# fraunhoferhhi/gaussian_gan_decoder

Measured on AMD Instinct MI355X. Metric: forward raster frames/s, 1M Gaussians @ 1024x1024, higher is better.
Workload: dtype f32; 1 GPU; 1000000 synthetic Gaussians ('cube' scene, seed 0, SH degree 0), 1024x1024, forward raster fp32, inputs resident in HBM; num_rendered=4152095, tiles=4096, parallelism=scene-parallel x1 (no collective)

## Files before the change

gaussian_gan_decoder_amd/csrc/ggd_lookback.inc:

```
constexpr uint32_t STATUS_PUB = 1u << 30, STATUS_COUNT_MASK = STATUS_PUB - 1u;
constexpr int LOOKBACK_BATCH = 16;

__device__ __forceinline__ uint32_t status_load(uint32_t* p) {
  return __hip_atomic_load(p, __ATOMIC_RELAXED, __HIP_MEMORY_SCOPE_AGENT);
}
__device__ __forceinline__ void status_store(uint32_t* p, uint32_t v) {
  __hip_atomic_store(p, v, __ATOMIC_RELAXED, __HIP_MEMORY_SCOPE_AGENT);
}

template <int STRIDE>
__device__ __forceinline__ uint32_t lookback_sum(uint32_t* p, int cnt) {
  uint32_t acc = 0;
  for (int b0 = 0; b0 < cnt; b0 += LOOKBACK_BATCH) {
    uint32_t v[LOOKBACK_BATCH];
#pragma unroll
    for (int i = 0; i < LOOKBACK_BATCH; ++i) v[i] = (b0 + i < cnt) ? status_load(p + (size_t)(b0 + i) * STRIDE) : STATUS_PUB;
#pragma unroll
    for (int i = 0; i < LOOKBACK_BATCH; ++i) {
      uint32_t x = v[i];
      if ((x >> 30) == 0u) {
        uint32_t* q = p + (size_t)(b0 + i) * STRIDE;
        do { __builtin_amdgcn_s_sleep(1); x = status_load(q); } while ((x >> 30) == 0u);
      }
      acc += x & STATUS_COUNT_MASK;
    }
  }
  return acc;
}

template <int STRIDE, typename TileT>
__device__ __forceinline__ uint32_t lookback_two_level(uint32_t* status, int col, int rows, TileT tile, int gshift, uint32_t local,
                                                       uint32_t start) {
  const int grp = (int)(tile >> gshift), mem = (int)(tile & (((TileT)1 << gshift) - (TileT)1));
  uint32_t* tile_words = status + col;
  uint32_t* group_words = status + (size_t)rows * STRIDE + col;
  status_store(tile_words + (size_t)tile * STRIDE, STATUS_PUB | local);
  const uint32_t in_group = lookback_sum<STRIDE>(tile_words + ((size_t)grp << gshift) * STRIDE, mem);
  if (mem == (1 << gshift) - 1) {
    const uint32_t aggregate = STATUS_PUB | (in_group + local);
    status_store(group_words + (size_t)grp * STRIDE, aggregate);
  }
  return start + in_group + lookback_sum<STRIDE>(group_words, grp);
}
```

gaussian_gan_decoder_amd/csrc/ggd_rowbin.hip:

```cpp
#include "ggd_common.h"

namespace {

#include "ggd_scan.inc"
#include "ggd_lookback.inc"

constexpr int RB_WAVES = RB_THREADS / 64;
constexpr int RB_STAGE = 4096;
constexpr int RB_STAGE1 = 4096;
constexpr int RB_WCHUNK = 64 * RB_IPL;

__device__ __forceinline__ void rb_write_row_tables(uint32_t* tab, int lane, uint32_t tot, uint32_t inc, uint32_t ent_cap) {
  const uint32_t rs = inc - tot;
  tab[RB_TAB_ROWSTART + lane] = rs;
  if (lane == 63) tab[RB_TAB_ROWSTART + 64] = inc;
  const uint32_t have = rs < ent_cap ? min(tot, ent_cap - rs) : 0u;
  const uint32_t nblk = (have + RB_CHUNK - 1) / RB_CHUNK;
  const uint32_t binc = wave_inclusive_scan(nblk);
  tab[RB_TAB_ROWBLK + lane] = binc - nblk;
  if (lane == 63) tab[RB_TAB_ROWBLK + 64] = binc;
  tab[RB_TAB_FLAG + lane] = 0u;
}

__global__ __launch_bounds__(RB_THREADS) void rb_count1_kernel(int W, int H, const uint2* __restrict__ rect,
                                                               const uint32_t* __restrict__ order,
                                                               const uint32_t* __restrict__ n_vis_ptr, int P,
                                                               uint2* __restrict__ packed, uint32_t* __restrict__ counts1,
                                                               const uint32_t* __restrict__ order_alt,
                                                               const uint32_t* __restrict__ use_alt) {
  __shared__ int diff[65];
  if (use_alt && *use_alt != 0u) order = order_alt;
  const uint32_t n_vis = min((uint32_t)P, *n_vis_ptr);
  const uint32_t base = (uint32_t)blockIdx.x * RB_CHUNK;
  if (base >= n_vis) return;
  const int tid = threadIdx.x;
  if (tid < 65) diff[tid] = 0;
  __syncthreads();
#pragma unroll
  for (int q = 0; q < RB_IPL; ++q) {
    const uint32_t rnk = base + (uint32_t)q * RB_THREADS + tid;
    if (rnk < n_vis) {
      const uint32_t id = order[rnk];
      const uint2 rc = rect[id];
      int x0 = (int)(rc.x & 0xffffu), x1 = (int)(rc.x >> 16), y0 = (int)(rc.y & 0xffffu), y1 = (int)(rc.y >> 16);
      const int n = (x1 - x0) * (y1 - y0);
      if (n <= 0) { x0 = x1 = y0 = y1 = 0; }
      packed[rnk] = make_uint2(id, (uint32_t)x0 | ((uint32_t)x1 << 8) | ((uint32_t)y0 << 16) | ((uint32_t)y1 << 24));
      if (n > 0) { atomicAdd(&diff[y0], 1); atomicAdd(&diff[y1], -1); }
    }
  }
  __syncthreads();
  if (tid < 64) counts1[(size_t)blockIdx.x * 64 + tid] = (uint32_t)wave_inclusive_scan(diff[tid]);
}

__global__ __launch_bounds__(1024) void rb_scan1_kernel(uint32_t* __restrict__ counts1,
                                                        const uint32_t* __restrict__ n_vis_ptr, int P,
                                                        uint32_t* __restrict__ tab, uint32_t ent_cap) {
  __shared__ uint32_t part[16][64];
  const int lane = threadIdx.x & 63, wv = threadIdx.x >> 6;
  const uint32_t n_vis = min((uint32_t)P, *n_vis_ptr);
  const int nb = (int)((n_vis + RB_CHUNK - 1) / RB_CHUNK);
  const int per = (nb + 15) / 16;
  const int r0 = min(nb, wv * per), r1 = min(nb, r0 + per);
  uint32_t s = 0;
#pragma unroll 8
  for (int r = r0; r < r1; ++r) s += counts1[(size_t)r * 64 + lane];
  part[wv][lane] = s;
  __syncthreads();
  uint32_t run = 0, tot = 0;
#pragma unroll
  for (int w = 0; w < 16; ++w) { const uint32_t p = part[w][lane]; if (w < wv) run += p; tot += p; }
#pragma unroll 8
  for (int r = r0; r < r1; ++r) {
    const size_t idx = (size_t)r * 64 + lane;
    const uint32_t c = counts1[idx];
    counts1[idx] = run;
    run += c;
  }
  if (wv == 0) rb_write_row_tables(tab, lane, tot, wave_inclusive_scan(tot), ent_cap);
}

template <int D, uint32_t M>
__device__ __forceinline__ void tr_stage(uint32_t& lo, uint32_t& hi, uint32_t lane) {
  const bool up = (lane & (uint32_t)D) != 0;
  const uint32_t keep = up ? ~M : M;
  const uint32_t slo = up ? ((lo & M) << D) : ((lo & ~M) >> D);
  const uint32_t shi = up ? ((hi & M) << D) : ((hi & ~M) >> D);
  lo = (lo & keep) | (uint32_t)__shfl_xor((int)slo, D, 64);
  hi = (hi & keep) | (uint32_t)__shfl_xor((int)shi, D, 64);
}

__device__ __forceinline__ uint64_t wave_transpose64(uint64_t row) {
  const uint32_t lane = threadIdx.x & 63;
  uint32_t lo = (uint32_t)row, hi = (uint32_t)(row >> 32);
  {
    const bool up = (lane & 32u) != 0;
    const uint32_t recv = (uint32_t)__shfl_xor((int)(up ? lo : hi), 32, 64);
    if (up) lo = recv; else hi = recv;
  }
  tr_stage<16, 0x0000FFFFu>(lo, hi, lane);
  tr_stage<8, 0x00FF00FFu>(lo, hi, lane);
  tr_stage<4, 0x0F0F0F0Fu>(lo, hi, lane);
  tr_stage<2, 0x33333333u>(lo, hi, lane);
  tr_stage<1, 0x55555555u>(lo, hi, lane);
  return (uint64_t)lo | ((uint64_t)hi << 32);
}

__device__ __forceinline__ uint32_t wave_cols(const uint32_t (&iv)[RB_IPL], int n_items, uint64_t (&cols)[RB_IPL]) {
  uint32_t cnt = 0;
#pragma unroll
  for (int q = 0; q < RB_IPL; ++q) {
    cols[q] = 0ull;
    if (q * 64 >= n_items) continue;
    const uint32_t l = iv[q] & 0xffu, h = iv[q] >> 8;
    const uint64_t below_h = h >= 64u ? ~0ull : ((1ull << h) - 1ull);
    const uint64_t row = h > l ? (below_h & ~((1ull << l) - 1ull)) : 0ull;
    cols[q] = wave_transpose64(row);
    cnt += (uint32_t)__popcll(cols[q]);
  }
  return cnt;
}

__device__ __forceinline__ bool rb_walk_items(uint32_t width, uint32_t fill) {
  const int wi = __ballot(width > 16u) ? 3 : (__ballot(width > 8u) ? 2 : (__ballot(width > 4u) ? 1 : 0));
  const int wf = __ballot(fill > 16u) ? 3 : (__ballot(fill > 8u) ? 2 : (__ballot(fill > 4u) ? 1 : 0));
  return wi <= wf + 1;
}

template <bool TWO, typename Emit>
__device__ __forceinline__ void wave_emit(const uint32_t (&iv)[RB_IPL], const uint32_t (&pa)[RB_IPL],
                                          const uint32_t (&pb)[RB_IPL], const uint64_t (&cols)[RB_IPL], int n_items,
                                          uint32_t& dst, uint4* slab , Emit&& emit) {
  const int lane = threadIdx.x & 63;
  const uint64_t lt_mask = (1ull << lane) - 1ull;
#pragma unroll
  for (int q = 0; q < RB_IPL; ++q) {
    if (q * 64 >= n_items) continue;
    __builtin_amdgcn_wave_barrier();
    slab[lane] = make_uint4((uint32_t)cols[q], (uint32_t)(cols[q] >> 32), dst, 0u);
    __builtin_amdgcn_wave_barrier();
    const uint32_t l = iv[q] & 0xffu, h = iv[q] >> 8;
    if (rb_walk_items(h > l ? h - l : 0u, (uint32_t)__popcll(cols[q]))) {
      for (uint32_t b = l; __ballot(b < h) != 0ull; ++b) {
        const bool act = b < h;
        const uint4 e = slab[act ? b : 0u];
        const uint64_t m = (uint64_t)e.x | ((uint64_t)e.y << 32);
        if (act) emit(e.z + (uint32_t)__popcll(m & lt_mask), pa[q], TWO ? pb[q] : 0u);
      }
      dst += (uint32_t)__popcll(cols[q]);
    } else {
      uint64_t col = cols[q];
      while (__ballot(col != 0ull) != 0ull) {
        const bool act = col != 0ull;
        const int k = act ? (__ffsll((unsigned long long)col) - 1) : 0;
        col &= col - 1ull;
        const uint32_t a = (uint32_t)__shfl((int)pa[q], k, 64);
        const uint32_t bb = TWO ? (uint32_t)__shfl((int)pb[q], k, 64) : 0u;
        if (act) { emit(dst, a, bb); dst += 1; }
      }
    }
  }
}

__global__ __launch_bounds__(RB_THREADS) void rb_scatter1_kernel(const uint2* __restrict__ packed,
                                                                 const uint32_t* __restrict__ n_vis_ptr, int P,
                                                                 const uint32_t* __restrict__ prefix1,
                                                                 const uint32_t* __restrict__ tab,
                                                                 uint2* __restrict__ ent, uint32_t ent_cap) {
  __shared__ uint4 slab[RB_WAVES][64];
  __shared__ uint32_t wcnt[RB_WAVES][64];
  const uint32_t n_vis = min((uint32_t)P, *n_vis_ptr);
  const uint32_t base = (uint32_t)blockIdx.x * RB_CHUNK;
  if (base >= n_vis) return;
  const int tid = threadIdx.x, lane = tid & 63, wv = tid >> 6;
  const uint32_t wbeg = base + (uint32_t)wv * RB_WCHUNK;
  const int n_items = (int)min((uint32_t)RB_WCHUNK, n_vis > wbeg ? n_vis - wbeg : 0u);
  uint32_t iv[RB_IPL], pa[RB_IPL], pb[RB_IPL];
#pragma unroll
  for (int q = 0; q < RB_IPL; ++q) {
    const int i = q * 64 + lane;
    uint2 it = make_uint2(0, 0);
    if (i < n_items) it = packed[wbeg + i];
    pa[q] = it.x; pb[q] = it.y & 0xffffu;
    iv[q] = it.y >> 16;
  }
  uint64_t cols[RB_IPL];
  const uint32_t mine = wave_cols(iv, n_items, cols);
  wcnt[wv][lane] = mine;
  __syncthreads();
  uint32_t dst = tab[RB_TAB_ROWSTART + lane] + prefix1[(size_t)blockIdx.x * 64 + lane];
#pragma unroll
  for (int w = 0; w < RB_WAVES; ++w) if (w < wv) dst += wcnt[w][lane];
  wave_emit<true>(iv, pa, pb, cols, n_items, dst, slab[wv], [&](uint32_t d, uint32_t id, uint32_t xx) {
    if (d < ent_cap) ent[d] = make_uint2(id, xx);
  });
}

__global__ __launch_bounds__(RB_THREADS) void rb_level1_kernel(const uint2* __restrict__ rect, const uint32_t* __restrict__ order,
                                                               const uint32_t* __restrict__ n_vis_ptr, int P,
                                                               const uint32_t* __restrict__ rowtot, uint32_t* status,
                                                               int chunks_max, int gshift_max, uint32_t* __restrict__ tab,
                                                               uint2* __restrict__ ent, uint32_t ent_cap,
                                                               const uint32_t* __restrict__ order_alt,
                                                               const uint32_t* __restrict__ use_alt,
                                                               const uint32_t* __restrict__ rowinst) {
  __shared__ uint4 slab[RB_WAVES][64];
  __shared__ uint32_t wcnt[RB_WAVES][64];
  __shared__ uint32_t s_base[64];
  __shared__ uint2 stage[RB_STAGE1];
  if (use_alt && *use_alt != 0u) order = order_alt;
  const uint32_t n_vis = min((uint32_t)P, *n_vis_ptr);
  const int tid = threadIdx.x, lane = tid & 63, wv = tid >> 6;
  uint32_t rowstart = 0;
  if (wv == 0) {
    uint32_t tot = 0;
#pragma unroll
    for (int r = 0; r < GGD_FOLD_REPS; ++r) tot += rowtot[r * 64 + lane];
    const uint32_t inc = wave_inclusive_scan(tot);
    rowstart = inc - tot;
    if (blockIdx.x == 0) {
      rb_write_row_tables(tab, lane, tot, inc, ent_cap);
      if (rowinst) {
        uint32_t inst = 0;
#pragma unroll
        for (int r = 0; r < GGD_FOLD_REPS; ++r) inst += rowinst[r * 64 + lane];
        tab[RB_TAB_ROWINST + lane] = inst;
      }
    }
  }
  const uint32_t base = (uint32_t)blockIdx.x * RB_CHUNK;
  if (base >= n_vis) return;
  const uint32_t wbeg = base + (uint32_t)wv * RB_WCHUNK;
  const int n_items = (int)min((uint32_t)RB_WCHUNK, n_vis > wbeg ? n_vis - wbeg : 0u);
  uint32_t iv[RB_IPL], pa[RB_IPL], pb[RB_IPL];
#pragma unroll
  for (int q = 0; q < RB_IPL; ++q) {
    const int i = q * 64 + lane;
    pa[q] = 0; pb[q] = 0; iv[q] = 0;
    if (i < n_items) {
      const uint32_t id = order[wbeg + i];
      const uint2 rc = rect[id];
      const uint32_t x0 = rc.x & 0xffffu, x1 = rc.x >> 16, y0 = rc.y & 0xffffu, y1 = rc.y >> 16;
      pa[q] = id;
      if ((int)(x1 - x0) * (int)(y1 - y0) > 0) { pb[q] = x0 | (x1 << 8); iv[q] = y0 | (y1 << 8); }
    }
  }
  uint64_t cols[RB_IPL];
  const uint32_t mine = wave_cols(iv, n_items, cols);
  wcnt[wv][lane] = mine;
  __syncthreads();
  if (wv == 0) {
    const uint32_t local = wcnt[0][lane] + wcnt[1][lane] + wcnt[2][lane] + wcnt[3][lane];
    const int chunk = (int)blockIdx.x;
    const int live = (int)((n_vis + RB_CHUNK - 1) / RB_CHUNK);
    const int gs = min(ggd_group_shift(live), gshift_max);
    s_base[lane] = lookback_two_level<64>(status, lane, chunks_max, chunk, gs, local, rowstart);
  }
  __syncthreads();
  uint32_t before = 0, rowtot_c = 0;
#pragma unroll
  for (int w = 0; w < RB_WAVES; ++w) { const uint32_t c = wcnt[w][lane]; if (w < wv) before += c; rowtot_c += c; }
  const uint32_t rowend = wave_inclusive_scan(rowtot_c);
  const uint32_t total = (uint32_t)__shfl((int)rowend, 63, 64);
  const uint32_t rowbeg = rowend - rowtot_c;
  const uint32_t gbase = s_base[lane];
  if (total <= (uint32_t)RB_STAGE1) {
    uint32_t ldst = rowbeg + before;
    wave_emit<true>(iv, pa, pb, cols, n_items, ldst, slab[wv], [&](uint32_t d, uint32_t id, uint32_t xx) { stage[d] = make_uint2(id, xx); });
    __syncthreads();
#pragma unroll 4
    for (int c = wv; c < 64; c += RB_WAVES) {
      const uint32_t n = (uint32_t)__shfl((int)rowtot_c, c, 64);
      if (n == 0) continue;
      const uint32_t b0 = (uint32_t)__shfl((int)rowbeg, c, 64), g = (uint32_t)__shfl((int)gbase, c, 64);
      for (uint32_t k = lane; k < n; k += 64) {
        const uint32_t d = g + k;
        if (d < ent_cap) ent[d] = stage[b0 + k];
      }
    }
    return;
  }
  uint32_t dst = gbase + before;
  wave_emit<true>(iv, pa, pb, cols, n_items, dst, slab[wv], [&](uint32_t d, uint32_t id, uint32_t xx) {
    if (d < ent_cap) ent[d] = make_uint2(id, xx);
  });
}

__device__ __forceinline__ bool rb_block_row_range(const uint32_t* __restrict__ tab, uint32_t blk, uint32_t ent_cap, int& row,
                                                   uint32_t& chunk, uint32_t& rbeg, uint32_t& rend) {
  const int lane = threadIdx.x & 63;
  const uint32_t first = tab[RB_TAB_ROWBLK + lane];
  const uint32_t total = tab[RB_TAB_ROWBLK + 64];
  const uint32_t start = tab[RB_TAB_ROWSTART + lane];
  const uint32_t all = tab[RB_TAB_ROWSTART + 64];
  if (blk >= total) return false;
  const int r = __popcll(__ballot(first <= blk)) - 1;
  row = r; chunk = blk - (uint32_t)__shfl((int)first, r, 64);
  rbeg = (uint32_t)__shfl((int)start, r, 64);
  rend = min(r == 63 ? all : (uint32_t)__shfl((int)start, (r + 1) & 63, 64), ent_cap);
  return true;
}

__global__ __launch_bounds__(RB_THREADS) void rb_count2_kernel(const uint2* __restrict__ ent, uint32_t ent_cap,
                                                               const uint32_t* __restrict__ tab,
                                                               uint32_t* __restrict__ counts2) {
  __shared__ int diff[65];
  int row; uint32_t chunk, rbeg, rend;
  if (!rb_block_row_range(tab, blockIdx.x, ent_cap, row, chunk, rbeg, rend)) return;
  const int tid = threadIdx.x;
  const uint32_t base = rbeg + chunk * RB_CHUNK;
  uint32_t xs[RB_IPL];
#pragma unroll
  for (int q = 0; q < RB_IPL; ++q) {
    const uint32_t i = base + (uint32_t)q * RB_THREADS + tid;
    xs[q] = i < rend ? ent[i].y : 0u;
  }
  if (tid < 65) diff[tid] = 0;
  __syncthreads();
#pragma unroll
  for (int q = 0; q < RB_IPL; ++q) {
    const uint32_t x0 = xs[q] & 0xffu, x1 = (xs[q] >> 8) & 0xffu;
    if (x1 > x0) { atomicAdd(&diff[x0], 1); atomicAdd(&diff[x1], -1); }
  }
  __syncthreads();
  if (tid < 64) counts2[(size_t)blockIdx.x * 64 + tid] = (uint32_t)wave_inclusive_scan(diff[tid]);
}

__global__ __launch_bounds__(1024) void rb_scan2_kernel(uint32_t* __restrict__ counts2, uint32_t* tab, int gx, int gy,
                                                        uint32_t* __restrict__ ranges) {
  __shared__ uint32_t part[16][64];
  const int lane = threadIdx.x & 63, wv = threadIdx.x >> 6;
  const int r = blockIdx.x;
  const uint32_t b0 = tab[RB_TAB_ROWBLK + r], b1 = tab[RB_TAB_ROWBLK + r + 1];
  const uint32_t nb = b1 - b0, per = (nb + 15u) / 16u;
  const uint32_t c0 = b0 + min(nb, (uint32_t)wv * per), c1 = min(b1, c0 + per);
  uint32_t s = 0;
#pragma unroll 4
  for (uint32_t b = c0; b < c1; ++b) s += counts2[(size_t)b * 64 + lane];
  part[wv][lane] = s;
  __syncthreads();
  uint32_t run = 0, tot = 0;
#pragma unroll
  for (int w = 0; w < 16; ++w) { const uint32_t p = part[w][lane]; if (w < wv) run += p; tot += p; }
#pragma unroll 4
  for (uint32_t b = c0; b < c1; ++b) {
    const size_t idx = (size_t)b * 64 + lane;
    const uint32_t c = counts2[idx];
    counts2[idx] = run;
    run += c;
  }
  if (wv == 0) {
    const uint32_t inc = wave_inclusive_scan(tot);
    if (lane == 63) {
      tab[RB_TAB_ROWINST + r] = inc;
      __builtin_amdgcn_fence(__ATOMIC_RELEASE, "agent");
      __hip_atomic_store(&tab[RB_TAB_FLAG + r], 1u, __ATOMIC_RELAXED, __HIP_MEMORY_SCOPE_AGENT);
    }
    uint32_t below = 0;
    if (lane < r) {
      while (__hip_atomic_load(&tab[RB_TAB_FLAG + lane], __ATOMIC_RELAXED, __HIP_MEMORY_SCOPE_AGENT) == 0u) {}
    }
    __builtin_amdgcn_fence(__ATOMIC_ACQUIRE, "agent");
    if (lane < r) below = __hip_atomic_load(&tab[RB_TAB_ROWINST + lane], __ATOMIC_RELAXED, __HIP_MEMORY_SCOPE_AGENT);
    const uint32_t binc = wave_inclusive_scan(below);
    const uint32_t rowbase = (uint32_t)__builtin_amdgcn_readlane((int)binc, 63);
    if (lane < gx) {
      const uint32_t start = rowbase + inc - tot;
      tab[RB_TAB_TILESTART + r * 64 + lane] = start;
      const int t = r * gx + lane;
      ranges[2 * t] = tot ? start : 0u;
      ranges[2 * t + 1] = tot ? start + tot : 0u;
    }
  }
}

template <bool SCAN>
__global__ __launch_bounds__(RB_THREADS) void rb_scatter2_kernel(const uint2* __restrict__ ent, uint32_t ent_cap,
                                                                 const uint32_t* __restrict__ tab,
                                                                 const uint32_t* __restrict__ prefix2,
                                                                 uint32_t* __restrict__ list, uint32_t capacity,
                                                                 uint32_t main_blocks, ggd_scan_piggy pg, int gx, int gy,
                                                                 uint32_t* __restrict__ ranges) {
  __shared__ uint4 slab[RB_WAVES][64];
  __shared__ uint32_t wcnt[RB_WAVES][64];
  __shared__ __attribute__((aligned(16))) uint32_t wsum[SCAN ? 2 * RB_WAVES : 1][64];
  __shared__ uint32_t stage[RB_STAGE];
  if (blockIdx.x >= main_blocks) {
    scan_apply_block(pg.in, pg.out, pg.n, pg.block_sums, (int)(blockIdx.x - main_blocks), stage, pg.sum_stride);
    return;
  }
  const int tid = threadIdx.x, lane = tid & 63, wv = tid >> 6;
  uint32_t rowinst = 0, rowblks = 0;
  if constexpr (SCAN) {
    rowinst = tab[RB_TAB_ROWINST + lane];
    rowblks = tab[RB_TAB_ROWBLK + lane + 1] - tab[RB_TAB_ROWBLK + lane];
    if ((int)blockIdx.x < gy && wv == 0) {
      const uint32_t nb_z = (uint32_t)__shfl((int)rowblks, (int)blockIdx.x, 64);
      if (nb_z == 0u && lane < gx) {
        const int t = (int)blockIdx.x * gx + lane;
        ranges[2 * t] = 0u;
        ranges[2 * t + 1] = 0u;
      }
    }
  }
  int row; uint32_t chunk, rbeg, rend;
  if (!rb_block_row_range(tab, blockIdx.x, ent_cap, row, chunk, rbeg, rend)) return;
  const uint32_t wbeg = rbeg + chunk * RB_CHUNK + (uint32_t)wv * RB_WCHUNK;
  const int n_items = (int)min((uint32_t)RB_WCHUNK, rend > wbeg ? rend - wbeg : 0u);
  uint32_t iv[RB_IPL], pa[RB_IPL], pb[RB_IPL];
  const uint32_t blkbeg = rbeg + chunk * RB_CHUNK;
  uint2 raw[RB_IPL];
#pragma unroll
  for (int q = 0; q < RB_IPL; ++q) {
    const int i = q * 64 + lane;
    raw[q] = ent[i < n_items ? wbeg + (uint32_t)i : blkbeg];
  }
  uint32_t gbase = 0;
  if constexpr (SCAN) {
    const uint32_t blk0 = blockIdx.x - chunk;
    const uint32_t nblk_row = (uint32_t)__shfl((int)rowblks, row, 64);
    constexpr int BATCH = 8;
    const uint32_t sub = (uint32_t)lane >> 4, c4 = ((uint32_t)lane & 15u) * 4u;
    uint4 bef4 = make_uint4(0, 0, 0, 0), tot4 = make_uint4(0, 0, 0, 0);
    for (uint32_t k0 = (uint32_t)wv * 4u; k0 < nblk_row; k0 += 4u * RB_WAVES * BATCH) {
      uint4 v[BATCH];
#pragma unroll
      for (int j = 0; j < BATCH; ++j) {
        const uint32_t k = k0 + sub + (uint32_t)(4 * RB_WAVES * j);
        v[j] = make_uint4(0, 0, 0, 0);
        if (k < nblk_row) v[j] = *reinterpret_cast<const uint4*>(prefix2 + (size_t)(blk0 + k) * 64 + c4);
      }
#pragma unroll
      for (int j = 0; j < BATCH; ++j) {
        const uint32_t k = k0 + sub + (uint32_t)(4 * RB_WAVES * j);
        tot4.x += v[j].x; tot4.y += v[j].y; tot4.z += v[j].z; tot4.w += v[j].w;
        const uint32_t m = k < chunk ? 0xffffffffu : 0u;
        bef4.x += v[j].x & m; bef4.y += v[j].y & m; bef4.z += v[j].z & m; bef4.w += v[j].w & m;
      }
    }
#pragma unroll
    for (int d = 16; d <= 32; d <<= 1) {
      tot4.x += (uint32_t)__shfl_xor((int)tot4.x, d, 64); tot4.y += (uint32_t)__shfl_xor((int)tot4.y, d, 64);
      tot4.z += (uint32_t)__shfl_xor((int)tot4.z, d, 64); tot4.w += (uint32_t)__shfl_xor((int)tot4.w, d, 64);
      bef4.x += (uint32_t)__shfl_xor((int)bef4.x, d, 64); bef4.y += (uint32_t)__shfl_xor((int)bef4.y, d, 64);
      bef4.z += (uint32_t)__shfl_xor((int)bef4.z, d, 64); bef4.w += (uint32_t)__shfl_xor((int)bef4.w, d, 64);
    }
    if (lane < 16) {
      *reinterpret_cast<uint4*>(&wsum[wv][c4]) = bef4;
      *reinterpret_cast<uint4*>(&wsum[RB_WAVES + wv][c4]) = tot4;
    }
  } else {
    gbase = tab[RB_TAB_TILESTART + row * 64 + lane] + prefix2[(size_t)blockIdx.x * 64 + lane];
  }
#pragma unroll
  for (int q = 0; q < RB_IPL; ++q) {
    const bool have = q * 64 + lane < n_items;
    pa[q] = have ? raw[q].x : 0u; pb[q] = 0;
    iv[q] = have ? raw[q].y & 0xffffu : 0u;
  }
  uint64_t cols[RB_IPL];
  const uint32_t mine = wave_cols(iv, n_items, cols);
  wcnt[wv][lane] = mine;
  __syncthreads();
  if constexpr (SCAN) {
    uint32_t bef = 0, tot = 0;
#pragma unroll
    for (int w = 0; w < RB_WAVES; ++w) { bef += wsum[w][lane]; tot += wsum[RB_WAVES + w][lane]; }
    const uint32_t rinc = wave_inclusive_scan(rowinst);
    const uint32_t rowbase = (uint32_t)__shfl((int)(rinc - rowinst), row, 64);
    const uint32_t start = rowbase + wave_inclusive_scan(tot) - tot;
    gbase = start + bef;
    if (chunk == 0u && wv == 0 && lane < gx) {
      const int t = row * gx + lane;
      ranges[2 * t] = tot ? start : 0u;
      ranges[2 * t + 1] = tot ? start + tot : 0u;
    }
  }
  uint32_t before = 0, coltot = 0;
#pragma unroll
  for (int w = 0; w < RB_WAVES; ++w) { const uint32_t c = wcnt[w][lane]; if (w < wv) before += c; coltot += c; }
  const uint32_t colend = wave_inclusive_scan(coltot);
  const uint32_t total = (uint32_t)__shfl((int)colend, 63, 64);
  const uint32_t colbeg = colend - coltot;
  if (total <= (uint32_t)RB_STAGE) {
    uint32_t ldst = colbeg + before;
    wave_emit<false>(iv, pa, pb, cols, n_items, ldst, slab[wv], [&](uint32_t d, uint32_t id, uint32_t) { stage[d] = id; });
    __syncthreads();
#pragma unroll 4
    for (int c = wv; c < 64; c += RB_WAVES) {
      const uint32_t n = (uint32_t)__shfl((int)coltot, c, 64);
      if (n == 0) continue;
      const uint32_t b0 = (uint32_t)__shfl((int)colbeg, c, 64), g = (uint32_t)__shfl((int)gbase, c, 64);
      for (uint32_t k = lane; k < n; k += 64) {
        const uint32_t d = g + k;
        if (d < capacity) list[d] = stage[b0 + k];
      }
    }
    return;
  }
  uint32_t dst = gbase + before;
  wave_emit<false>(iv, pa, pb, cols, n_items, dst, slab[wv], [&](uint32_t d, uint32_t id, uint32_t) {
    if (d < capacity) list[d] = id;
  });
}

#include "ggd_rowbin_wide.inc"

}

bool ggd_rowbin_supported(int W, int H) { return W > 0 && H > 0 && (W + 15) / 16 <= 255 && (H + 15) / 16 <= 255; }

int ggd_launch_rowbin(ggd_ctx* ctx, hipStream_t s, const ggd_params& prm, const uint2* rect, const uint32_t* order,
                      const uint32_t* n_vis_ptr, uint32_t* list, uint32_t* ranges, uint32_t capacity, void* tmp,
                      size_t tmp_bytes, const uint32_t* order_alt, const uint32_t* use_alt, const ggd_scan_piggy* apply,
                      const uint32_t* fold_rowtot, uint32_t* fold_status1, const uint32_t* fold_rowinst, bool* scan_in_scatter) {
  if (scan_in_scatter) *scan_in_scatter = false;
  if (!ggd_rowbin_supported(prm.width, prm.height)) return ggd_fail(ctx, GGD_E_INVALID, "tile grid too large for row binning");
  const ggd_rowbin_tmp lay = ggd_rowbin_layout(prm.P, capacity, prm.width, prm.height);
  if (tmp_bytes < lay.total) return ggd_fail(ctx, GGD_E_INVALID, "rowbin tmp too small");
  const int gx = (prm.width + 15) / 16, gy = (prm.height + 15) / 16;
  const bool wide = rb_is_wide(prm.width, prm.height);
  char* p = static_cast<char*>(tmp);
  uint2* packed = reinterpret_cast<uint2*>(p + lay.packed);
  uint32_t* counts1 = reinterpret_cast<uint32_t*>(p + lay.counts1);
  uint32_t* tab = reinterpret_cast<uint32_t*>(p + lay.tab);
  uint2* ent = reinterpret_cast<uint2*>(p + lay.ent);
  uint32_t* counts2 = reinterpret_cast<uint32_t*>(p + lay.counts2);
  const int nb1 = rb_blocks1(prm.P);
  const uint32_t nb2 = rb_blocks2(capacity, wide);
  const uint32_t nb_apply = apply ? (uint32_t)apply->nb : 0u;
  const ggd_scan_piggy pg = apply ? *apply : ggd_scan_piggy{};
  static_assert(RB_THREADS == SCAN_THREADS, "the appended scan workgroups share the launch's block size");
  if (wide) {
    const int ngy = (gy + 63) / 64, ngx = (gx + 63) / 64, nby = 64 * ngy, nbx = 64 * ngx;
    hipLaunchKernelGGL(rbw_count1_kernel, dim3(nb1), dim3(RB_THREADS), 0, s, rect, order, n_vis_ptr, prm.P, nby, packed,
                       counts1, order_alt, use_alt);
    hipLaunchKernelGGL(rbw_scan1_kernel, dim3(1), dim3(1024), 0, s, counts1, n_vis_ptr, prm.P, ngy, tab, capacity);
    hipLaunchKernelGGL(rbw_scatter1_kernel, dim3(nb1), dim3(RB_THREADS), 0, s, packed, n_vis_ptr, prm.P, ngy, counts1, tab,
                       ent, capacity);
    hipLaunchKernelGGL(rbw_count2_kernel, dim3(nb2), dim3(RB_THREADS), 0, s, ent, capacity, tab, nbx, counts2);
    hipLaunchKernelGGL(rbw_scan2_kernel, dim3(gy), dim3(1024), 0, s, counts2, tab, gx, gy, ngx, ranges);
    hipLaunchKernelGGL(rbw_scatter2_kernel, dim3(nb2 + nb_apply), dim3(RB_THREADS), 0, s, ent, capacity, tab, ngx, counts2, list,
                       capacity, nb2, pg);
    GGD_HIP(hipGetLastError());
    return GGD_OK;
  }
  const bool fused2 = fold_rowtot && fold_status1 && fold_rowinst && nb2 <= RB_SCAN_IN_SCATTER_MAX_BLOCKS;
  if (fold_rowtot && fold_status1) {
    hipLaunchKernelGGL(rb_level1_kernel, dim3(nb1), dim3(RB_THREADS), 0, s, rect, order, n_vis_ptr, prm.P, fold_rowtot,
                       fold_status1, nb1, ggd_group_shift(nb1), tab, ent, capacity, order_alt, use_alt,
                       fused2 ? fold_rowinst : nullptr);
  } else {
    hipLaunchKernelGGL(rb_count1_kernel, dim3(nb1), dim3(RB_THREADS), 0, s, prm.width, prm.height, rect, order,
                       n_vis_ptr, prm.P, packed, counts1, order_alt, use_alt);
    hipLaunchKernelGGL(rb_scan1_kernel, dim3(1), dim3(1024), 0, s, counts1, n_vis_ptr, prm.P, tab, capacity);
    hipLaunchKernelGGL(rb_scatter1_kernel, dim3(nb1), dim3(RB_THREADS), 0, s, packed, n_vis_ptr, prm.P, counts1, tab,
                       ent, capacity);
  }
  hipLaunchKernelGGL(rb_count2_kernel, dim3(nb2), dim3(RB_THREADS), 0, s, ent, capacity, tab, counts2);
  if (fused2) {
    hipLaunchKernelGGL(rb_scatter2_kernel<true>, dim3(nb2 + nb_apply), dim3(RB_THREADS), 0, s, ent, capacity, tab, counts2, list,
                       capacity, nb2, pg, gx, gy, ranges);
    if (scan_in_scatter) *scan_in_scatter = true;
  } else {
    hipLaunchKernelGGL(rb_scan2_kernel, dim3(gy), dim3(1024), 0, s, counts2, tab, gx, gy, ranges);
    hipLaunchKernelGGL(rb_scatter2_kernel<false>, dim3(nb2 + nb_apply), dim3(RB_THREADS), 0, s, ent, capacity, tab, counts2, list,
                       capacity, nb2, pg, gx, gy, ranges);
  }
  GGD_HIP(hipGetLastError());
  return GGD_OK;
}
```

Measured before the change: 5122 frames/s.

## Overlap decoupled lookback with staging emit in rowbin level-1 kernel

Splits the two-level lookback so each block publishes its own group prefix early, issues the loads for earlier group aggregates, and only settles them after emitting entries into shared staging. This hides the lookback latency behind the emit work. The change also hoists the order/rect loads ahead of the row-table scan, moves the early-exit path to the top, and batches the staging-to-global copy loop four rows at a time using readlane. Risks: more register pressure from the held aggregate batch and the prefetched rects, and a subtle ordering dependency on publishing before waiting.

```diff
diff --git a/gaussian_gan_decoder_amd/csrc/ggd_lookback.inc b/gaussian_gan_decoder_amd/csrc/ggd_lookback.inc
--- a/gaussian_gan_decoder_amd/csrc/ggd_lookback.inc
+++ b/gaussian_gan_decoder_amd/csrc/ggd_lookback.inc
@@ -9,28 +9,48 @@
 }
 
 template <int STRIDE>
+__device__ __forceinline__ void lookback_request(uint32_t* p, int cnt, int b0, uint32_t (&v)[LOOKBACK_BATCH]) {
+#pragma unroll
+  for (int i = 0; i < LOOKBACK_BATCH; ++i) v[i] = (b0 + i < cnt) ? status_load(p + (size_t)(b0 + i) * STRIDE) : STATUS_PUB;
+}
+template <int STRIDE>
+__device__ __forceinline__ uint32_t lookback_settle(uint32_t* p, int b0, const uint32_t (&v)[LOOKBACK_BATCH]) {
+  uint32_t acc = 0;
+#pragma unroll
+  for (int i = 0; i < LOOKBACK_BATCH; ++i) {
+    uint32_t x = v[i];
+    if ((x >> 30) == 0u) {
+      uint32_t* q = p + (size_t)(b0 + i) * STRIDE;
+      do { __builtin_amdgcn_s_sleep(1); x = status_load(q); } while ((x >> 30) == 0u);
+    }
+    acc += x & STATUS_COUNT_MASK;
+  }
+  return acc;
+}
+template <int STRIDE>
 __device__ __forceinline__ uint32_t lookback_sum(uint32_t* p, int cnt) {
   uint32_t acc = 0;
   for (int b0 = 0; b0 < cnt; b0 += LOOKBACK_BATCH) {
     uint32_t v[LOOKBACK_BATCH];
-#pragma unroll
-    for (int i = 0; i < LOOKBACK_BATCH; ++i) v[i] = (b0 + i < cnt) ? status_load(p + (size_t)(b0 + i) * STRIDE) : STATUS_PUB;
-#pragma unroll
-    for (int i = 0; i < LOOKBACK_BATCH; ++i) {
-      uint32_t x = v[i];
-      if ((x >> 30) == 0u) {
-        uint32_t* q = p + (size_t)(b0 + i) * STRIDE;
-        do { __builtin_amdgcn_s_sleep(1); x = status_load(q); } while ((x >> 30) == 0u);
-      }
-      acc += x & STATUS_COUNT_MASK;
-    }
+    lookback_request<STRIDE>(p, cnt, b0, v);
+    acc += lookback_settle<STRIDE>(p, b0, v);
   }
+  return acc;
+}
+template <int STRIDE>
+__device__ __forceinline__ uint32_t lookback_sum_finish(uint32_t* p, int cnt, uint32_t (&v)[LOOKBACK_BATCH]) {
+  uint32_t acc = 0;
+  int b0 = 0;
+  do {
+    if (b0 != 0) lookback_request<STRIDE>(p, cnt, b0, v);
+    acc += lookback_settle<STRIDE>(p, b0, v);
+    b0 += LOOKBACK_BATCH;
+  } while (b0 < cnt);
   return acc;
 }
 
 template <int STRIDE, typename TileT>
-__device__ __forceinline__ uint32_t lookback_two_level(uint32_t* status, int col, int rows, TileT tile, int gshift, uint32_t local,
-                                                       uint32_t start) {
+__device__ __forceinline__ uint32_t lookback_own_group(uint32_t* status, int col, int rows, TileT tile, int gshift, uint32_t local) {
   const int grp = (int)(tile >> gshift), mem = (int)(tile & (((TileT)1 << gshift) - (TileT)1));
   uint32_t* tile_words = status + col;
   uint32_t* group_words = status + (size_t)rows * STRIDE + col;
@@ -40,5 +60,25 @@
     const uint32_t aggregate = STATUS_PUB | (in_group + local);
     status_store(group_words + (size_t)grp * STRIDE, aggregate);
   }
-  return start + in_group + lookback_sum<STRIDE>(group_words, grp);
+  return in_group;
 }
+template <int STRIDE, typename TileT>
+__device__ __forceinline__ void lookback_groups_request(uint32_t* status, int col, int rows, TileT tile, int gshift,
+                                                        uint32_t (&v)[LOOKBACK_BATCH]) {
+  lookback_request<STRIDE>(status + (size_t)rows * STRIDE + col, (int)(tile >> gshift), 0, v);
+}
+template <int STRIDE, typename TileT>
+__device__ __forceinline__ uint32_t lookback_groups_finish(uint32_t* status, int col, int rows, TileT tile, int gshift,
+                                                           uint32_t (&v)[LOOKBACK_BATCH]) {
+  return lookback_sum_finish<STRIDE>(status + (size_t)rows * STRIDE + col, (int)(tile >> gshift), v);
+}
+template <int STRIDE, typename TileT>
+__device__ __forceinline__ uint32_t lookback_earlier_groups(uint32_t* status, int col, int rows, TileT tile, int gshift) {
+  return lookback_sum<STRIDE>(status + (size_t)rows * STRIDE + col, (int)(tile >> gshift));
+}
+template <int STRIDE, typename TileT>
+__device__ __forceinline__ uint32_t lookback_two_level(uint32_t* status, int col, int rows, TileT tile, int gshift, uint32_t local,
+                                                       uint32_t start) {
+  const uint32_t in_group = lookback_own_group<STRIDE>(status, col, rows, tile, gshift, local);
+  return start + in_group + lookback_earlier_groups<STRIDE>(status, col, rows, tile, gshift);
+}
diff --git a/gaussian_gan_decoder_amd/csrc/ggd_rowbin.hip b/gaussian_gan_decoder_amd/csrc/ggd_rowbin.hip
--- a/gaussian_gan_decoder_amd/csrc/ggd_rowbin.hip
+++ b/gaussian_gan_decoder_amd/csrc/ggd_rowbin.hip
@@ -208,79 +208,126 @@
   __shared__ uint32_t wcnt[RB_WAVES][64];
   __shared__ uint32_t s_base[64];
   __shared__ uint2 stage[RB_STAGE1];
-  if (use_alt && *use_alt != 0u) order = order_alt;
-  const uint32_t n_vis = min((uint32_t)P, *n_vis_ptr);
-  const int tid = threadIdx.x, lane = tid & 63, wv = tid >> 6;
+  const uint32_t nv_word = *n_vis_ptr;
+  const uint32_t alt_word = *(use_alt ? use_alt : n_vis_ptr);
+  asm volatile("" : : "s"(nv_word), "s"(alt_word));
+  if (use_alt && alt_word != 0u) order = order_alt;
+  const uint32_t n_vis = min((uint32_t)P, nv_word);
+  const int tid = threadIdx.x, lane = tid & 63, wv = __builtin_amdgcn_readfirstlane(tid >> 6);
+  const uint32_t base = (uint32_t)blockIdx.x * RB_CHUNK;
+  if (base >= n_vis) {
+    if (blockIdx.x == 0 && wv == 0) {
+      uint32_t tot = 0, inst = 0;
+#pragma unroll
+      for (int r = 0; r < GGD_FOLD_REPS; ++r) tot += rowtot[r * 64 + lane];
+      rb_write_row_tables(tab, lane, tot, wave_inclusive_scan(tot), ent_cap);
+      if (rowinst) {
+#pragma unroll
+        for (int r = 0; r < GGD_FOLD_REPS; ++r) inst += rowinst[r * 64 + lane];
+        tab[RB_TAB_ROWINST + lane] = inst;
+      }
+    }
+    return;
+  }
+  const uint32_t wbeg = base + (uint32_t)wv * RB_WCHUNK;
+  const int n_items = (int)min((uint32_t)RB_WCHUNK, n_vis > wbeg ? n_vis - wbeg : 0u);
+  const bool tables = blockIdx.x == 0;
+  uint32_t rt[GGD_FOLD_REPS], ri[GGD_FOLD_REPS];
+  if (wv == 0) {
+#pragma unroll
+    for (int r = 0; r < GGD_FOLD_REPS; ++r) rt[r] = rowtot[r * 64 + lane];
+    if (tables && rowinst) {
+#pragma unroll
+      for (int r = 0; r < GGD_FOLD_REPS; ++r) ri[r] = rowinst[r * 64 + lane];
+    }
+  }
+  uint32_t ids[RB_IPL];
+  uint2 rcs[RB_IPL];
+#pragma unroll
+  for (int q = 0; q < RB_IPL; ++q) ids[q] = order[min(wbeg + (uint32_t)(q * 64 + lane), n_vis - 1u)];
+#pragma unroll
+  for (int q = 0; q < RB_IPL; ++q) rcs[q] = rect[ids[q]];
   uint32_t rowstart = 0;
   if (wv == 0) {
     uint32_t tot = 0;
 #pragma unroll
-    for (int r = 0; r < GGD_FOLD_REPS; ++r) tot += rowtot[r * 64 + lane];
+    for (int r = 0; r < GGD_FOLD_REPS; ++r) tot += rt[r];
     const uint32_t inc = wave_inclusive_scan(tot);
     rowstart = inc - tot;
-    if (blockIdx.x == 0) {
+    if (tables) {
       rb_write_row_tables(tab, lane, tot, inc, ent_cap);
       if (rowinst) {
         uint32_t inst = 0;
 #pragma unroll
-        for (int r = 0; r < GGD_FOLD_REPS; ++r) inst += rowinst[r * 64 + lane];
+        for (int r = 0; r < GGD_FOLD_REPS; ++r) inst += ri[r];
         tab[RB_TAB_ROWINST + lane] = inst;
       }
     }
   }
-  const uint32_t base = (uint32_t)blockIdx.x * RB_CHUNK;
-  if (base >= n_vis) return;
-  const uint32_t wbeg = base + (uint32_t)wv * RB_WCHUNK;
-  const int n_items = (int)min((uint32_t)RB_WCHUNK, n_vis > wbeg ? n_vis - wbeg : 0u);
   uint32_t iv[RB_IPL], pa[RB_IPL], pb[RB_IPL];
 #pragma unroll
   for (int q = 0; q < RB_IPL; ++q) {
-    const int i = q * 64 + lane;
-    pa[q] = 0; pb[q] = 0; iv[q] = 0;
-    if (i < n_items) {
-      const uint32_t id = order[wbeg + i];
-      const uint2 rc = rect[id];
-      const uint32_t x0 = rc.x & 0xffffu, x1 = rc.x >> 16, y0 = rc.y & 0xffffu, y1 = rc.y >> 16;
-      pa[q] = id;
-      if ((int)(x1 - x0) * (int)(y1 - y0) > 0) { pb[q] = x0 | (x1 << 8); iv[q] = y0 | (y1 << 8); }
-    }
+    const bool have = q * 64 + lane < n_items;
+    const uint32_t x0 = rcs[q].x & 0xffffu, x1 = rcs[q].x >> 16, y0 = rcs[q].y & 0xffffu, y1 = rcs[q].y >> 16;
+    const bool area = have && (int)(x1 - x0) * (int)(y1 - y0) > 0;
+    pa[q] = have ? ids[q] : 0u;
+    pb[q] = area ? x0 | (x1 << 8) : 0u;
+    iv[q] = area ? y0 | (y1 << 8) : 0u;
   }
   uint64_t cols[RB_IPL];
   const uint32_t mine = wave_cols(iv, n_items, cols);
   wcnt[wv][lane] = mine;
   __syncthreads();
-  if (wv == 0) {
-    const uint32_t local = wcnt[0][lane] + wcnt[1][lane] + wcnt[2][lane] + wcnt[3][lane];
-    const int chunk = (int)blockIdx.x;
-    const int live = (int)((n_vis + RB_CHUNK - 1) / RB_CHUNK);
-    const int gs = min(ggd_group_shift(live), gshift_max);
-    s_base[lane] = lookback_two_level<64>(status, lane, chunks_max, chunk, gs, local, rowstart);
-  }
-  __syncthreads();
   uint32_t before = 0, rowtot_c = 0;
 #pragma unroll
   for (int w = 0; w < RB_WAVES; ++w) { const uint32_t c = wcnt[w][lane]; if (w < wv) before += c; rowtot_c += c; }
+  const int chunk = (int)blockIdx.x;
+  const int live = (int)((n_vis + RB_CHUNK - 1) / RB_CHUNK);
+  const int gs = min(ggd_group_shift(live), gshift_max);
+  uint32_t in_group = 0;
+  if (wv == 0) in_group = lookback_own_group<64>(status, lane, chunks_max, chunk, gs, rowtot_c);
   const uint32_t rowend = wave_inclusive_scan(rowtot_c);
   const uint32_t total = (uint32_t)__shfl((int)rowend, 63, 64);
   const uint32_t rowbeg = rowend - rowtot_c;
-  const uint32_t gbase = s_base[lane];
   if (total <= (uint32_t)RB_STAGE1) {
+    uint32_t agg[LOOKBACK_BATCH];
+    if (wv == 0) lookback_groups_request<64>(status, lane, chunks_max, chunk, gs, agg);
     uint32_t ldst = rowbeg + before;
     wave_emit<true>(iv, pa, pb, cols, n_items, ldst, slab[wv], [&](uint32_t d, uint32_t id, uint32_t xx) { stage[d] = make_uint2(id, xx); });
+    if (wv == 0) s_base[lane] = rowstart + in_group + lookback_groups_finish<64>(status, lane, chunks_max, chunk, gs, agg);
     __syncthreads();
-#pragma unroll 4
-    for (int c = wv; c < 64; c += RB_WAVES) {
-      const uint32_t n = (uint32_t)__shfl((int)rowtot_c, c, 64);
-      if (n == 0) continue;
-      const uint32_t b0 = (uint32_t)__shfl((int)rowbeg, c, 64), g = (uint32_t)__shfl((int)gbase, c, 64);
-      for (uint32_t k = lane; k < n; k += 64) {
-        const uint32_t d = g + k;
-        if (d < ent_cap) ent[d] = stage[b0 + k];
+    const uint32_t gbase = s_base[lane];
+#pragma unroll 1
+    for (int c0 = wv; c0 < 64; c0 += 4 * RB_WAVES) {
+      uint32_t n[4], b0[4], g[4];
+      uint2 e[4];
+#pragma unroll
+      for (int j = 0; j < 4; ++j) {
+        const int c = c0 + j * RB_WAVES;
+        n[j] = (uint32_t)__builtin_amdgcn_readlane((int)rowtot_c, c);
+        b0[j] = (uint32_t)__builtin_amdgcn_readlane((int)rowbeg, c);
+        g[j] = (uint32_t)__builtin_amdgcn_readlane((int)gbase, c);
+      }
+#pragma unroll
+      for (int j = 0; j < 4; ++j) e[j] = stage[min(b0[j] + (uint32_t)lane, (uint32_t)(RB_STAGE1 - 1))];
+#pragma unroll
+      for (int j = 0; j < 4; ++j) {
+        const uint32_t d = g[j] + (uint32_t)lane;
+        if ((uint32_t)lane < n[j] && d < ent_cap) ent[d] = e[j];
+      }
+#pragma unroll
+      for (int j = 0; j < 4; ++j) {
+        for (uint32_t k = (uint32_t)lane + 64u; k < n[j]; k += 64) {
+          const uint32_t d = g[j] + k;
+          if (d < ent_cap) ent[d] = stage[b0[j] + k];
+        }
       }
     }
     return;
   }
-  uint32_t dst = gbase + before;
+  if (wv == 0) s_base[lane] = rowstart + in_group + lookback_earlier_groups<64>(status, lane, chunks_max, chunk, gs);
+  __syncthreads();
+  uint32_t dst = s_base[lane] + before;
   wave_emit<true>(iv, pa, pb, cols, n_items, dst, slab[wv], [&](uint32_t d, uint32_t id, uint32_t xx) {
     if (d < ent_cap) ent[d] = make_uint2(id, xx);
   });
```

Measured after the change: 4938 frames/s. -3.6%, worse.
